# microsoft/DFOL-VQA

Hardware: AMD Instinct MI355X
Metric: questions/sec (GQA programs, N=100 objects) (higher is better)
Workload: dtype f32

## Files before the change

### dfol_vqa_amd/csrc/dfol_pair_h2.hip

```cpp
#include "dfol_common.h"
#include "dfol_split.h"

#include <stdlib.h>

#include <type_traits>

#ifdef DFOL_PAIR_TRACE
__device__ long long dfol_h2_trace_buf[8 * 8 * 64];
#define TRACE(slot)                                                                                                  \
    do {                                                                                                             \
        if (trace_on && lane == 0) dfol_h2_trace_buf[(trace_blk * 8 + wave) * 64 + (slot)] = clock64();              \
    } while (0)
#else
#define TRACE(slot)
#endif

#ifndef DFOL_H2_PREFETCH
#define DFOL_H2_PREFETCH 1
#endif
#ifndef DFOL_H2_BDEPTH
#define DFOL_H2_BDEPTH 2
#endif
#ifndef DFOL_H1_BDEPTH
#define DFOL_H1_BDEPTH 4
// ... 35 lines not shown
    return r;
}

__global__ void h2_row_scale_kernel(const float* __restrict__ W2, int64_t ld_w2, int HID2, int HID1, float* __restrict__ tail) {
    const int lane = threadIdx.x & 63, r = blockIdx.x * (blockDim.x >> 6) + (threadIdx.x >> 6);
    if (r >= H2_ROWS) return;
    float m = 0.f;
    if (r < HID2)
        for (int k = lane; k < HID1; k += 64) m = fmaxf(m, fabsf(W2[(int64_t)r * ld_w2 + k] * H2_LN2));
#pragma unroll
    for (int s = 32; s >= 1; s >>= 1) m = fmaxf(m, __shfl_xor(m, s, 64));
    const int e = dfol_scale_exp(m);
    if (lane == 0) {
        tail[r] = ldexpf(H2_NL2E, -e);
        reinterpret_cast<int32_t*>(tail)[H2_ROWS + r] = e;
    }
}

template <int NP>
__global__ void h2_pack_w2_kernel(const float* __restrict__ W2, int64_t ld_w2, int HID2, int HID1, const float* __restrict__ tail,
                                  u32x4* __restrict__ out) {
    constexpr int PIECES = NP * H2_ROWS * 4;
    const int idx = blockIdx.x * blockDim.x + threadIdx.x;
    if (idx >= (HID1 / H2_CH) * PIECES) return;
    const int c = idx / PIECES, rem = idx - c * PIECES;
    const int p = rem / (H2_ROWS * 4), rr = rem - p * H2_ROWS * 4, r = rr >> 2, slot = rr & 3;
    const int kq = slot ^ dfol_swz(r);
    const int e = reinterpret_cast<const int32_t*>(tail)[H2_ROWS + r];
    uint32_t piece[4];
#pragma unroll
    for (int j = 0; j < 4; ++j) {
        float w0 = 0.f, w1 = 0.f;
        if (r < HID2) {
            w0 = ldexpf(W2[(int64_t)r * ld_w2 + c * H2_CH + h2_kperm(kq, 2 * j)] * H2_LN2, e);
            w1 = ldexpf(W2[(int64_t)r * ld_w2 + c * H2_CH + h2_kperm(kq, 2 * j + 1)] * H2_LN2, e);
        }
        uint32_t h, l;
        dfol_split2h(w0, w1, h, l);
        piece[j] = p == 0 ? h : l;
    }
    out[idx] = u32x4{piece[0], piece[1], piece[2], piece[3]};
}

struct H2Train {
    float* Z;
    float* pre2;
    int64_t ld_pre2;
    float* geo;
    float* x;
    int64_t ld_x;
    const int64_t* pair_off;
};

template <int NB16, bool TBF16, bool TRAIN = false, int NP = 2>
__global__ __launch_bounds__(512) __attribute__((amdgpu_waves_per_eu(2, 2))) void pair_ll32h_kernel(
    const float* UV_ , int64_t ld_uv_, int HID1, const float* __restrict__ pos_, int64_t ld_pos_,
    const float* __restrict__ Wg_, const u32x4* __restrict__ W2h_, const float* __restrict__ b2_, int HID2,
    const float* __restrict__ E_, int64_t ld_e, const float* __restrict__ be, const int32_t* __restrict__ n_obj,
    const int32_t* __restrict__ obj_off, int Q, int tiles_per_image, int wg_tiles, const int32_t* __restrict__ req_col,
    const int32_t* __restrict__ req_tile, const uint8_t* __restrict__ req_orient, int K, int NS, float dflt,
    void* __restrict__ tiles_v, H2Train tr) {
    constexpr int MT = 2, WAVES = 8;
    constexpr int ROWS = NB16 * 16, T = WAVES * 64, SLOTS = MT * 16 * WAVES;
    static_assert(NB16 > 16 && NB16 <= H2_TILES, "geometry");
    static_assert(NP == 2 || (NP == 1 && !TRAIN), "pieces per operand (the train forward keeps both)");
    constexpr int PIECES = NP * H2_ROWS * 4;
    __shared__ __attribute__((aligned(16))) u32x4 Bs[2 * PIECES];
    __shared__ __attribute__((aligned(16))) u32x4 WgA[(256 / H2_CH) * 2 * 64];
    constexpr int STAGE_FLOATS = 8192;
    __shared__ __attribute__((aligned(16))) float stage[STAGE_FLOATS];

    const int wave = __builtin_amdgcn_readfirstlane((int)threadIdx.x >> 6);
#ifdef DFOL_PAIR_TRACE
    const int trace_b0 = 3000 / wg_tiles, trace_step = 500 / wg_tiles > 0 ? 500 / wg_tiles : 1;
    const int trace_blk = ((int)blockIdx.x - trace_b0) / trace_step;
    const bool trace_on = (int)blockIdx.x >= trace_b0 && ((int)blockIdx.x - trace_b0) % trace_step == 0 && trace_blk < 8;
#endif
    const int nchunk = HID1 / H2_CH, lastc = nchunk - 1;
    const int tile_end = (int)min((int64_t)blockIdx.x * wg_tiles + wg_tiles, (int64_t)Q * tiles_per_image);
    auto dma_chunk0_all = [&](const u32x4* W2h) __attribute__((always_inline)) {
        int tid = threadIdx.x;
        asm volatile("" : "+v"(tid));
#pragma unroll
        for (int i = 0; i < (PIECES + T - 1) / T; ++i)
            if (PIECES % T == 0 || T * i + wave * 64 < PIECES)
                __builtin_amdgcn_global_load_lds(W2h + T * i + tid, (__attribute__((address_space(3))) void*)&Bs[T * i + wave * 64], 16, 0, 0);
    };
    bool started = false;
    bool b0 = false;
    int stage_q = -1;
    for (int tile = (int)blockIdx.x * wg_tiles; tile < tile_end; tile = TRAIN ? tile_end : tile + 1) {
        const int q = tile / tiles_per_image, tb = tile - q * tiles_per_image;
        const int n = n_obj[q], npairs = n * (n - 1);
        if (tb * SLOTS >= npairs) continue;
        bool any = TRAIN;
        for (int k = 0; k < K; ++k) any |= req_col[(int64_t)k * Q + q] >= 0;
        if (!any) continue;
        const int64_t prow0 = TRAIN ? tr.pair_off[q] : 0;
        const u32x4* W2h = W2h_;
        const float *Wg = Wg_, *b2 = b2_, *E = E_, *UV = UV_, *pos = pos_;
        int64_t ld_uv = ld_uv_, ld_pos = ld_pos_;
        asm volatile("" : "+s"(W2h), "+s"(Wg), "+s"(b2), "+s"(E));
        asm volatile("" : "+s"(UV), "+s"(pos), "+s"(ld_uv), "+s"(ld_pos));
        int tid = threadIdx.x;
        asm volatile("" : "+v"(tid));
        const int lane = tid & 63, kh = lane >> 4, r16 = lane & 15;
        const float* cf = reinterpret_cast<const float*>(W2h + (int64_t)nchunk * PIECES);

        TRACE(0);
        if (!started) dma_chunk0_all(W2h);
        const int first = obj_off[q];
        u32x4 geoB[MT];
        const char* img_uv = reinterpret_cast<const char*>(UV + (int64_t)first * ld_uv);
        uint32_t uoff[MT], voff[MT];
        uint32_t zoff[MT];
        auto slot_geometry = [&]() __attribute__((always_inline)) {
#pragma unroll
            for (int m = 0; m < MT; ++m) {
                const int e_slot = tb * SLOTS + wave * (MT * 16) + m * 16 + r16;
                const bool valid = e_slot < npairs;
                zoff[m] = (TRAIN && valid) ? (uint32_t)(e_slot * HID1 + 4 * kh) * 4u : 0xffffffffu;
                const int s = valid ? e_slot / (n - 1) : 0, oo_ = valid ? e_slot - s * (n - 1) : 0, o = oo_ + (oo_ >= s);
                const float4 g = dfol_pair_geometry(pos + (int64_t)(first + s) * ld_pos, pos + (int64_t)(first + o) * ld_pos);
                uint32_t gh01, gl01, gh23, gl23;
                dfol_split2h(g.x, g.y, gh01, gl01);
                dfol_split2h(g.z, g.w, gh23, gl23);
                if (TRAIN && valid && kh == 0) *reinterpret_cast<floatx4*>(tr.geo + (prow0 + e_slot) * 4) = floatx4{g.x, g.y, g.z, g.w};
                geoB[m] = kh == 0 ? u32x4{gh01, gh23, gl01, gl23} : (kh == 1 ? u32x4{gh01, gh23, 0u, 0u} : u32x4{0u, 0u, 0u, 0u});
                uoff[m] = (uint32_t)(s * (int)ld_uv + 4 * kh) * 4u;
                voff[m] = (uint32_t)(o * (int)ld_uv + HID1 + 4 * kh) * 4u;
            }
        };
        constexpr int SR = STAGE_FLOATS / ROWS - 2;
        const int Kc = K < SR ? K : SR;
        floatx4 acc[MT][NB16];
#pragma unroll
        for (int m = 0; m < MT; ++m)
#pragma unroll
            for (int i = 0; i < NB16; ++i) acc[m][i] = floatx4{0.f, 0.f, 0.f, 0.f};

        auto dma_chunk = [&](int c, int buf, int w, int ln) __attribute__((always_inline)) {
            constexpr int PER_WAVE = PIECES / 4;
            const u32x4* src = W2h + (int64_t)c * PIECES + w * PER_WAVE + ln;
            u32x4* dst = &Bs[buf * PIECES + w * PER_WAVE];
#pragma unroll
            for (int g = 0; g < PER_WAVE / 64; g += 4) {
#if DFOL_H2_DMA_ASM
                const uint32_t d = (uint32_t)(uintptr_t)(__attribute__((address_space(3))) void*)(dst + 64 * g);
                const u32x4* sp = src + 64 * g;
#pragma clang diagnostic push
#pragma clang diagnostic ignored "-Winline-asm"
                const uint32_t m0v = __builtin_amdgcn_readfirstlane(d);
                const int rem = PER_WAVE / 64 - g;
                if (rem >= 4)
                    asm volatile("s_mov_b32 m0, %1\n\ts_nop 0\n\tglobal_load_lds_dwordx4 %0, off\n\tglobal_load_lds_dwordx4 %0, off offset:1024\n\t"
                                 "global_load_lds_dwordx4 %0, off offset:2048\n\tglobal_load_lds_dwordx4 %0, off offset:3072" ::"v"(sp), "s"(m0v) : "memory", "m0");
                else if (rem == 3)
                    asm volatile("s_mov_b32 m0, %1\n\ts_nop 0\n\tglobal_load_lds_dwordx4 %0, off\n\tglobal_load_lds_dwordx4 %0, off offset:1024\n\t"
                                 "global_load_lds_dwordx4 %0, off offset:2048" ::"v"(sp), "s"(m0v) : "memory", "m0");
                else if (rem == 2)
                    asm volatile("s_mov_b32 m0, %1\n\ts_nop 0\n\tglobal_load_lds_dwordx4 %0, off\n\tglobal_load_lds_dwordx4 %0, off offset:1024" ::"v"(sp), "s"(m0v) : "memory", "m0");
                else
                    asm volatile("s_mov_b32 m0, %1\n\ts_nop 0\n\tglobal_load_lds_dwordx4 %0, off" ::"v"(sp), "s"(m0v) : "memory", "m0");
#pragma clang diagnostic pop
#else
                auto d = (__attribute__((address_space(3))) void*)(dst + 64 * g);
                __builtin_amdgcn_global_load_lds(src + 64 * g, d, 16, 0, 0);
                if (g + 1 < PER_WAVE / 64) __builtin_amdgcn_global_load_lds(src + 64 * g, d, 16, 1024, 0);
                if (g + 2 < PER_WAVE / 64) __builtin_amdgcn_global_load_lds(src + 64 * g, d, 16, 2048, 0);
                if (g + 3 < PER_WAVE / 64) __builtin_amdgcn_global_load_lds(src + 64 * g, d, 16, 3072, 0);
#endif
            }
        };
        floatx4 ru[MT][2], rv[MT][2];
        auto load_uv = [&](int c) __attribute__((always_inline)) {
            const char* base = img_uv + (uint32_t)__builtin_amdgcn_readfirstlane(H2_CH * 4 * c);
#pragma unroll
            for (int m = 0; m < MT; ++m)
#pragma unroll
                for (int half = 0; half < 2; ++half) {
                    ru[m][half] = *reinterpret_cast<const floatx4*>(base + uoff[m] + 64 * half);
                    rv[m][half] = *reinterpret_cast<const floatx4*>(base + voff[m] + 64 * half);
                }
        };
        u32x4 ap[MT][NP];
        auto make_a = [&](int c) __attribute__((always_inline)) {
            floatx4 z[MT][2];
#pragma unroll
            for (int t = 0; t < 2; ++t) {
                const f16x8 wa = __builtin_bit_cast(f16x8, WgA[(2 * c + t) * 64 + lane]);
#pragma unroll
                for (int m = 0; m < MT; ++m)
                    z[m][t] = __builtin_amdgcn_mfma_f32_16x16x32_f16(wa, __builtin_bit_cast(f16x8, geoB[m]), ru[m][t] + rv[m][t], 0, 0, 0);
            }
#pragma unroll
            for (int m = 0; m < MT; ++m)
#pragma unroll
                for (int t = 0; t < 2; ++t)
#pragma unroll
                    for (int jp = 0; jp < 2; ++jp) {
                        const float z0 = z[m][t][2 * jp], z1 = z[m][t][2 * jp + 1];
                        const float a0 = __builtin_amdgcn_fmed3f(z0, h2_elu_neg(z0), H2_AMAX);
                        const float a1 = __builtin_amdgcn_fmed3f(z1, h2_elu_neg(z1), H2_AMAX);
                        const uint32_t hh = __builtin_bit_cast(uint32_t, __builtin_convertvector((f32x2){a0, a1}, f16x2));
                        ap[m][0][2 * t + jp] = hh;
                        if constexpr (NP == 2)
                            ap[m][1][2 * t + jp] = __builtin_bit_cast(uint32_t, __builtin_convertvector((f32x2){h2_resid<false>(a0, hh), h2_resid<true>(a1, hh)}, f16x2));
                        if (TRAIN) z[m][t][2 * jp] = a0 * H2_LN2, z[m][t][2 * jp + 1] = a1 * H2_LN2;
                    }
            if (TRAIN && !(DFOL_H2T_SKIP & 1)) {
                char* zimg = reinterpret_cast<char*>(tr.Z + prow0 * HID1) + (uint32_t)__builtin_amdgcn_readfirstlane(H2_CH * 4 * c);
#pragma unroll
                for (int m = 0; m < MT; ++m)
                    if (zoff[m] != 0xffffffffu) {
#pragma unroll
                        for (int t = 0; t < 2; ++t) *reinterpret_cast<floatx4*>(zimg + zoff[m] + 64 * t) = z[m][t];
                    }
            }
        };
        const int boff = r16 * 4 + (kh ^ dfol_swz(r16));
        int bbase = boff;
        auto load_b = [&](int i, f16x8 (&b)[NP]) __attribute__((always_inline)) {
#pragma unroll
            for (int p = 0; p < NP; ++p) b[p] = __builtin_bit_cast(f16x8, Bs[bbase + i * 64 + p * H2_ROWS * 4]);
        };
        constexpr int PA3[3] = {1, 0, 0}, PB3[3] = {0, 1, 0};
        auto chunk_mfma = [&]() __attribute__((always_inline)) {
            constexpr int D = NP == 2 ? DFOL_H2_BDEPTH : DFOL_H1_BDEPTH;
            f16x8 bq[D + 1][NP];
#pragma unroll
            for (int d = 0; d < D; ++d) load_b(d, bq[d]);
#pragma unroll
            for (int i = 0; i < NB16; ++i) {
                if (i + D < NB16) load_b(i + D, bq[(i + D) % (D + 1)]);
                __builtin_amdgcn_sched_barrier(0);
#pragma unroll
                for (int m = 0; m < MT; ++m) {
#pragma unroll
                    for (int x = NP == 2 ? 0 : 2; x < 3; ++x)
                        acc[m][i] = __builtin_amdgcn_mfma_f32_16x16x32_f16(__builtin_bit_cast(f16x8, ap[m][PA3[x]]), bq[i % (D + 1)][PB3[x]], acc[m][i], 0, 0, 0);
                    __builtin_amdgcn_sched_barrier(0);
                }
            }
        };
        slot_geometry();
        if (started) {
            __syncthreads();
            if (!b0) dma_chunk0_all(W2h);
        } else {
            int tid = threadIdx.x;
            asm volatile("" : "+v"(tid));
            for (int i = tid; i < (HID1 / 16) * 64; i += T) {
                const int kt = i >> 6, ln = i & 63, khh = ln >> 4;
                u32x4 frag = {0u, 0u, 0u, 0u};
                if (khh < 2) {
                    const float4 g = *reinterpret_cast<const float4*>(Wg + (kt * 16 + (ln & 15)) * 4);
                    uint32_t h01, l01, h23, l23;
                    dfol_split2h(g.x * H2_L2E, g.y * H2_L2E, h01, l01);
                    dfol_split2h(g.z * H2_L2E, g.w * H2_L2E, h23, l23);
                    frag = khh == 0 ? u32x4{h01, h23, h01, h23} : u32x4{l01, l23, 0u, 0u};
                }
                WgA[i] = frag;
            }
        }
        if (q != stage_q) {
            int tid = threadIdx.x;
            asm volatile("" : "+v"(tid));
            for (int i = tid; i < ROWS; i += T) {
                stage[i] = H2_NL2E * (i < HID2 ? b2[i] : -1.0e30f);
                stage[ROWS + i] = i < HID2 ? cf[i] : 0.f;
            }
            for (int k = 0; k < Kc; ++k) {
                const int col = req_col[(int64_t)k * Q + q];
                for (int i = tid; i < ROWS; i += T) stage[ROWS * (2 + k) + i] = (col >= 0 && i < HID2) ? E[(int64_t)col * ld_e + i] : 0.f;
            }
        }
        __builtin_amdgcn_s_waitcnt(0x0F70);
        __syncthreads();

        const bool pf = (lastc & 1) && tile + 1 < tile_end;
        auto run_half = [&](auto y_tag) __attribute__((always_inline)) {
            constexpr bool Y = decltype(y_tag)::value;
            TRACE(1);
            if (Y) {
                if (nchunk > 1) dma_chunk(1, 1, wave - 4, lane);
                if (DFOL_H2_PREFETCH) load_uv(0);
                __syncthreads();
            } else if (DFOL_H2_PREFETCH) {
                load_uv(0);
            }
            TRACE(2);
            for (int c = 0; c < nchunk; ++c) {
                if (!DFOL_H2_PREFETCH) load_uv(c);
                if (DFOL_H2_PREFETCH) {
                    floatx4 t0 = ru[0][0], t1 = ru[0][1], t2 = ru[1][0], t3 = ru[1][1], t4 = rv[0][0], t5 = rv[0][1], t6 = rv[1][0], t7 = rv[1][1];
                    asm volatile("s_waitcnt vmcnt(0)" : "+v"(t0), "+v"(t1), "+v"(t2), "+v"(t3), "+v"(t4), "+v"(t5), "+v"(t6), "+v"(t7));
                    ru[0][0] = t0, ru[0][1] = t1, ru[1][0] = t2, ru[1][1] = t3, rv[0][0] = t4, rv[0][1] = t5, rv[1][0] = t6, rv[1][1] = t7;
                }
                TRACE(40 + c);
                if (Y && !DFOL_H2_DMA_LATE && c >= 1 && c < lastc) dma_chunk(c + 1, (c + 1) & 1, wave - 4, lane);
                TRACE(50 + c);
                make_a(c);
#pragma unroll
                for (int m = 0; m < MT; ++m)
#pragma unroll
                    for (int p = 0; p < NP; ++p) asm volatile("" : "+v"(ap[m][p]));
                __builtin_amdgcn_sched_barrier(0);
                if (Y && DFOL_H2_DMA_LATE && c >= 1 && c < lastc) dma_chunk(c + 1, (c + 1) & 1, wave - 4, lane);
                TRACE(3 + 4 * c);
                __syncthreads();
                __builtin_amdgcn_sched_barrier(0);
                TRACE(4 + 4 * c);
                bbase = boff + (c & 1) * PIECES;
                if (DFOL_H2_PREFETCH && c < lastc) load_uv(c + 1);
                chunk_mfma();
                if (Y) __builtin_amdgcn_s_waitcnt(0x0F70);
                TRACE(5 + 4 * c);
                if (!Y || c < lastc) __syncthreads();
                TRACE(6 + 4 * c);
            }
            if (!Y && pf) {
                int ln = lane;
                asm volatile("" : "+v"(ln));
                dma_chunk(0, 0, wave, ln);
            }
        };
        if (wave < 4) run_half(std::false_type());
        else run_half(std::true_type());

        const int64_t tile_sz = (int64_t)NS * NS;
#pragma unroll
        for (int m = 0; m < MT; ++m)
#pragma unroll
            for (int i = 0; i < NB16; ++i) {
                const float bv = stage[i * 16 + r16], cm = stage[ROWS + i * 16 + r16];
                if (TRAIN && !(DFOL_H2T_SKIP & 2)) {
                    const int colp = i * 16 + r16;
#pragma unroll
                    for (int e = 0; e < 4; ++e) {
                        const int ee = tb * SLOTS + wave * (MT * 16) + m * 16 + 4 * kh + e;
                        if (colp < HID2 && ee < npairs)
                            *reinterpret_cast<float*>(reinterpret_cast<char*>(tr.pre2 + prow0 * tr.ld_pre2) + (uint32_t)(ee * (int)tr.ld_pre2 + colp) * 4u) =
                                -H2_LN2 * fmaf(acc[m][i][e], cm, bv);
                    }
                }
#pragma unroll
                for (int e = 0; e < 4; ++e) acc[m][i][e] = __builtin_amdgcn_rcpf(1.0f + __builtin_amdgcn_exp2f(fmaf(acc[m][i][e], cm, bv)));
            }
        for (int k = 0; k < K; ++k) {
            const int col = req_col[(int64_t)k * Q + q];
            if (col < 0) continue;
            float vm[MT];
#pragma unroll
            for (int m = 0; m < MT; ++m) {
                float part[4] = {0.f, 0.f, 0.f, 0.f};
                if (k < Kc) {
                    const float* erow = stage + ROWS * (2 + k) + r16;
#pragma unroll
                    for (int i = 0; i < NB16; ++i) {
                        const float ev = erow[i * 16];
#pragma unroll
                        for (int e = 0; e < 4; ++e) part[e] = fmaf(acc[m][i][e], ev, part[e]);
                    }
                } else {
                    const float* erow = E + (int64_t)col * ld_e;
                    int c16 = r16;
                    asm volatile("" : "+v"(c16));
#pragma unroll
                    for (int i = 0; i < NB16; ++i) {
                        const float ev = erow[min(i * 16 + c16, HID2 - 1)];
#pragma unroll
                        for (int e = 0; e < 4; ++e) part[e] = fmaf(acc[m][i][e], ev, part[e]);
                    }
                }
#pragma unroll
                for (int e = 0; e < 4; ++e) part[e] = dfol_group_sum<16>(part[e]);
                vm[m] = r16 == 0 ? part[0] : (r16 == 1 ? part[1] : (r16 == 2 ? part[2] : part[3]));
            }
            const float shifted = __int_as_float(__builtin_amdgcn_update_dpp(0, __float_as_int(vm[1]), 0x114, 0xF, 0xF, false));
            if (r16 < 8) {
                const int hi = r16 >> 2;
                const float v = hi ? shifted : vm[0];
                const int ee = tb * SLOTS + wave * (MT * 16) + hi * 16 + 4 * kh + (r16 & 3);
                if (ee < npairs) {
                    if (TRAIN) {
                        tr.x[(int64_t)k * tr.ld_x + prow0 + ee] = v;
                        continue;
                    }
                    int ss, oo;
                    dfol_offdiag_slot_rcp(ee, n, ss, oo);
                    const float x = v + (be ? be[col] : 0.f);
                    const float val = fminf(x, 0.f) - dfol_log(1.0f + dfol_exp(-fabsf(x)));
                    const int64_t at = (int64_t)req_tile[(int64_t)k * Q + q] * tile_sz +
                                       ((req_orient && req_orient[(int64_t)k * Q + q]) ? (int64_t)oo * NS + ss : (int64_t)ss * NS + oo);
                    if (TBF16) {
                        uint32_t u = __float_as_uint(val);
                        u += 0x7fffu + ((u >> 16) & 1u);
                        reinterpret_cast<uint16_t*>(tiles_v)[at] = (uint16_t)(u >> 16);
                    } else {
                        reinterpret_cast<float*>(tiles_v)[at] = val;
                    }
                }
            }
        }
        TRACE(60);
        started = true;
        stage_q = q;
        b0 = pf;
    }
    __builtin_amdgcn_s_waitcnt(0x0F70);
}

__global__ __launch_bounds__(512) void h2_uv_range_kernel(const float* __restrict__ UV, int64_t ld_uv, int HID1, const float* __restrict__ pos,
                                                          int64_t ld_pos, const float* __restrict__ Wg, const int32_t* __restrict__ n_obj,
                                                          const int32_t* __restrict__ obj_off, uint32_t* __restrict__ status) {
    __shared__ float4 part[512];
    __shared__ float box[4][8];
    const int q = blockIdx.x, n = n_obj[q], first = obj_off[q], t = threadIdx.x, lane = t & 63, wave = t >> 6;
    if (n < 2) return;
    const int G = (2 * HID1) / 4, R = 512 / G, cg = t % G, rg = t / G;
    float4 m = {-INFINITY, -INFINITY, -INFINITY, -INFINITY};
    bool nan = false;
    const float* base = UV + (int64_t)first * ld_uv + 4 * cg;
    auto take = [&](const float4 a) {
        nan |= (a.x != a.x) | (a.y != a.y) | (a.z != a.z) | (a.w != a.w);
        m.x = fmaxf(m.x, a.x), m.y = fmaxf(m.y, a.y), m.z = fmaxf(m.z, a.z), m.w = fmaxf(m.w, a.w);
    };
    int o = rg;
    for (; o + 3 * R < n; o += 4 * R) {
        const float4 a = *reinterpret_cast<const float4*>(base + (int64_t)o * ld_uv), b = *reinterpret_cast<const float4*>(base + (int64_t)(o + R) * ld_uv);
        const float4 c = *reinterpret_cast<const float4*>(base + (int64_t)(o + 2 * R) * ld_uv), d = *reinterpret_cast<const float4*>(base + (int64_t)(o + 3 * R) * ld_uv);
        take(a), take(b), take(c), take(d);
    }
    for (; o < n; o += R) take(*reinterpret_cast<const float4*>(base + (int64_t)o * ld_uv));
    if (nan) m.x = NAN;
    part[t] = m;
    float lox = INFINITY, hix = -INFINITY, loy = INFINITY, hiy = -INFINITY;
    for (int i = t; i < n; i += 512) {
        const float* p = pos + (int64_t)(first + i) * ld_pos;
        const float cx = p[0] + p[2] / 2.0f, cy = p[1] + p[3] / 2.0f;
        lox = fminf(lox, cx), hix = fmaxf(hix, cx), loy = fminf(loy, cy), hiy = fmaxf(hiy, cy);
    }
#pragma unroll
    for (int s = 32; s >= 1; s >>= 1) {
        lox = fminf(lox, __shfl_xor(lox, s, 64)), hix = fmaxf(hix, __shfl_xor(hix, s, 64));
        loy = fminf(loy, __shfl_xor(loy, s, 64)), hiy = fmaxf(hiy, __shfl_xor(hiy, s, 64));
    }
    if (lane == 0) box[0][wave] = lox, box[1][wave] = hix, box[2][wave] = loy, box[3][wave] = hiy;
    __syncthreads();
    if (t < HID1) {
#pragma unroll
        for (int w = 0; w < 8; ++w) lox = fminf(lox, box[0][w]), hix = fmaxf(hix, box[1][w]), loy = fminf(loy, box[2][w]), hiy = fmaxf(hiy, box[3][w]);
        const float* pf = reinterpret_cast<const float*>(part);
        float mu = -INFINITY, mv = -INFINITY;
        bool bad = false;
        for (int r = 0; r < R; ++r) {
            const float u = pf[(r * G + t / 4) * 4 + (t & 3)], v = pf[(r * G + (HID1 + t) / 4) * 4 + (t & 3)];
            const float ux = pf[(r * G + t / 4) * 4], vx = pf[(r * G + (HID1 + t) / 4) * 4];
            bad |= (ux != ux) | (vx != vx);
            mu = fmaxf(mu, u), mv = fmaxf(mv, v);
        }
        const float dmax = sqrtf((hix - lox) * (hix - lox) + (hiy - loy) * (hiy - loy));
        const float4 g = *reinterpret_cast<const float4*>(Wg + t * 4);
        const float geo = H2_L2E * (fabsf(g.x) * dmax + fabsf(g.y) * 1.57079632679489661923f + fabsf(g.z) + fabsf(g.w));
        const float bound = mu + mv + geo;
// ... 156 lines not shown
        }
        __syncthreads();
        for (int j = 0; j < n_ent; ++j) {
            const int first = __builtin_amdgcn_readfirstlane(ent[2][j]), end = __builtin_amdgcn_readfirstlane(ent[3][j]);
            if (end <= w0 || first >= w0 + MT * 16) continue;
            const int p = __builtin_amdgcn_readfirstlane(ent[0][j]), col = __builtin_amdgcn_readfirstlane(ent[1][j]);
            float vm[MT];
#pragma unroll
            for (int m = 0; m < MT; ++m) {
                float part[4] = {0.f, 0.f, 0.f, 0.f};
                if (j < SR) {
                    const float* erow = stage + ROWS * (2 + j) + r16;
#pragma unroll
                    for (int i = 0; i < NB16; ++i) {
                        const float ev = erow[i * 16];
#pragma unroll
                        for (int e = 0; e < 4; ++e) part[e] = fmaf(acc[m][i][e], ev, part[e]);
                    }
                } else {
                    const float* erow = E + (int64_t)col * ld_e;
#pragma unroll
                    for (int i = 0; i < NB16; ++i) {
                        const float ev = i * 16 + r16 < HID2 ? erow[i * 16 + r16] : 0.f;
#pragma unroll
                        for (int e = 0; e < 4; ++e) part[e] = fmaf(acc[m][i][e], ev, part[e]);
                    }
                }
#pragma unroll
                for (int e = 0; e < 4; ++e) part[e] = dfol_group_sum<16>(part[e]);
                vm[m] = r16 == 0 ? part[0] : (r16 == 1 ? part[1] : (r16 == 2 ? part[2] : part[3]));
            }
            const float shifted = __int_as_float(__builtin_amdgcn_update_dpp(0, __float_as_int(vm[1]), 0x114, 0xF, 0xF, false));
            if (r16 < 8) {
                const int hi = r16 >> 2;
                const int g = w0 + hi * 16 + 4 * kh + (r16 & 3);
                if (g >= first && g < end && g - first < NS) {
                    const float x = (hi ? shifted : vm[0]) + (be ? be[col] : 0.f);
                    ll[(int64_t)p * NS + (g - first)] = fminf(x, 0.f) - log1pf(expf(-fabsf(x)));
                }
            }
        }
    }
}

}

#ifdef DFOL_PAIR_TRACE
extern "C" int dfol_pair_h2_trace_read(long long* out) { return (int)hipMemcpyFromSymbol(out, HIP_SYMBOL(dfol_h2_trace_buf), sizeof(dfol_h2_trace_buf)); }
#endif

#ifndef DFOL_H2_WG_TILES
#define DFOL_H2_WG_TILES 4
#endif
static int h2_wg_tiles() {
    const char* e = getenv("DFOL_PAIR_TILES");
    const int t = e ? atoi(e) : DFOL_H2_WG_TILES;
    return t < 1 ? 1 : (t > 64 ? 64 : t);
}

extern "C" int64_t dfol_pair_w2_f16x2_bytes(int32_t HID1) { return (int64_t)(HID1 / H2_CH) * H2_PIECES * 16 + 2 * H2_ROWS * 4; }
extern "C" int64_t dfol_pair_w2_f16_bytes(int32_t HID1) { return (int64_t)(HID1 / H2_CH) * H1_PIECES * 16 + 2 * H2_ROWS * 4; }

template <int NP>
static int h2_pack_w2(const char* name, const float* W2, int64_t ld_w2, int32_t HID2, int32_t HID1, void* W2_split, void* stream) {
    DFOL_REQUIRE(HID1 > 0 && HID1 <= 256 && HID1 % H2_CH == 0, "%s: HID1=%d must be a multiple of %d, <= 256", name, HID1, H2_CH);
    DFOL_REQUIRE(HID2 > 256 && HID2 <= 320, "%s: HID2=%d must be in (256, 320]", name, HID2);
    DFOL_REQUIRE(W2 && W2_split && ld_w2 >= HID1, "%s: null pointer or ld_w2 < HID1", name);
    DFOL_REQUIRE((uintptr_t)W2_split % 16 == 0, "%s: output must be 16-byte aligned", name);
    const int total = (HID1 / H2_CH) * NP * H2_ROWS * 4;
    float* tail = reinterpret_cast<float*>(reinterpret_cast<u32x4*>(W2_split) + total);
    hipLaunchKernelGGL(h2_row_scale_kernel, dim3(H2_ROWS / 4), dim3(256), 0, (hipStream_t)stream, W2, ld_w2, HID2, HID1, tail);
    hipLaunchKernelGGL(h2_pack_w2_kernel<NP>, dim3(dfol_cdiv(total, 256)), dim3(256), 0, (hipStream_t)stream, W2, ld_w2, HID2, HID1, (const float*)tail,
                       (u32x4*)W2_split);
    DFOL_LAUNCH_CHECK(name);
    return 0;
}

extern "C" int dfol_pair_pack_w2_f16x2(const float* W2, int64_t ld_w2, int32_t HID2, int32_t HID1, void* W2_split, void* stream) {
    return h2_pack_w2<2>("pair_pack_w2_f16x2", W2, ld_w2, HID2, HID1, W2_split, stream);
}

extern "C" int dfol_pair_pack_w2_f16(const float* W2, int64_t ld_w2, int32_t HID2, int32_t HID1, void* W2_split, void* stream) {
    return h2_pack_w2<1>("pair_pack_w2_f16", W2, ld_w2, HID2, HID1, W2_split, stream);
}

template <int NP>
static int h2_pair_ll(const char* name, const float* UV, int64_t ld_uv, int32_t HID1, const float* pos, int64_t ld_pos, const float* Wg,
                      const void* W2_split, const float* b2, int32_t HID2, const float* E, int64_t ld_e, const float* be, const int32_t* n_obj,
                      const int32_t* obj_off, int32_t Q, int32_t max_n, const int32_t* req_col, const int32_t* req_tile, const uint8_t* req_orient,
                      int32_t K, int32_t NS, float default_ll, int32_t tile_dtype, void* tiles_v, void* stream) {
    DFOL_REQUIRE(tile_dtype == DFOL_TILE_F32 || (tile_dtype == DFOL_TILE_BF16 && NS % 8 == 0), "%s: tile_dtype=%d (bf16 tiles need NS %% 8 == 0)", name, tile_dtype);
    DFOL_REQUIRE(Q >= 0 && K >= 0 && NS > 0 && NS % 4 == 0 && max_n >= 0 && max_n <= NS, "%s: bad sizes Q=%d K=%d NS=%d max_n=%d", name, Q, K, NS, max_n);
    DFOL_REQUIRE(HID1 > 0 && HID1 <= 256 && HID1 % H2_CH == 0 && ld_uv % 4 == 0, "%s: HID1=%d must be a multiple of %d, <= 256, UV rows 16-byte aligned", name, HID1, H2_CH);
    DFOL_REQUIRE(HID2 > 256 && HID2 <= 320, "%s: HID2=%d must be in (256, 320]", name, HID2);
    DFOL_REQUIRE(max_n <= DFOL_OFFDIAG_RCP_MAX_N, "%s: max_n=%d is above %d objects per image, the range of the epilogue's reciprocal pair decode (dfol_common.h)",
                 name, max_n, DFOL_OFFDIAG_RCP_MAX_N);
    if (Q == 0 || K == 0 || max_n < 2) return 0;
    DFOL_REQUIRE(UV && pos && Wg && W2_split && b2 && E && n_obj && obj_off && req_col && req_tile && tiles_v, "%s: null pointer", name);
    DFOL_REQUIRE(((uintptr_t)UV % 16 == 0) && ((uintptr_t)W2_split % 16 == 0) && ((uintptr_t)Wg % 16 == 0), "%s: operands must be 16-byte aligned", name);
    hipStream_t st = (hipStream_t)stream;
    const int tpi = dfol_cdiv((int64_t)max_n * (max_n - 1), 256);
    DFOL_REQUIRE((int64_t)Q * tpi < ((int64_t)1 << 31), "%s: too many tiles", name);
    DFOL_REQUIRE((int64_t)max_n * ld_uv * 4 < ((int64_t)1 << 31), "%s: an image's U / V rows must span less than 2 GB", name);
    const int wgt = h2_wg_tiles();
    const dim3 grid((unsigned)dfol_cdiv((int64_t)Q * tpi, wgt));
    if (uint32_t* status = dfol_range_status_ptr())
        hipLaunchKernelGGL(h2_uv_range_kernel, dim3((unsigned)Q), dim3(512), 0, st, UV, ld_uv, HID1, pos, ld_pos, Wg, n_obj, obj_off, status);
    const H2Train none = {nullptr, nullptr, 0, nullptr, nullptr, 0, nullptr};
#define DFOL_PAIR32H(NBV, BF)                                                                                                       \
    hipLaunchKernelGGL((pair_ll32h_kernel<NBV, BF, false, NP>), grid, dim3(512), 0, st, UV, ld_uv, HID1, pos, ld_pos, Wg, (const u32x4*)W2_split, b2, HID2, \
                       E, ld_e, be, n_obj, obj_off, Q, tpi, wgt, req_col, req_tile, req_orient, K, NS, default_ll, tiles_v, none)
    if (HID2 <= 272) { if (tile_dtype == DFOL_TILE_BF16) DFOL_PAIR32H(17, true); else DFOL_PAIR32H(17, false); }
    else if (HID2 <= 288) { if (tile_dtype == DFOL_TILE_BF16) DFOL_PAIR32H(18, true); else DFOL_PAIR32H(18, false); }
    else if (HID2 <= 304) { if (tile_dtype == DFOL_TILE_BF16) DFOL_PAIR32H(19, true); else DFOL_PAIR32H(19, false); }
    else { if (tile_dtype == DFOL_TILE_BF16) DFOL_PAIR32H(20, true); else DFOL_PAIR32H(20, false); }
#undef DFOL_PAIR32H
    DFOL_LAUNCH_CHECK(name);
    return 0;
}

extern "C" int dfol_pair_ll_h2_f32(const float* UV, int64_t ld_uv, int32_t HID1, const float* pos, int64_t ld_pos, const float* Wg,
                                   const void* W2_split, const float* b2, int32_t HID2, const float* E, int64_t ld_e,
                                   const float* be, const int32_t* n_obj, const int32_t* obj_off, int32_t Q, int32_t max_n,
                                   const int32_t* req_col, const int32_t* req_tile, const uint8_t* req_orient, int32_t K,
                                   int32_t NS, float default_ll, int32_t tile_dtype, void* tiles_v, void* stream) {
    return h2_pair_ll<2>("pair_ll_h2", UV, ld_uv, HID1, pos, ld_pos, Wg, W2_split, b2, HID2, E, ld_e, be, n_obj, obj_off, Q, max_n, req_col, req_tile, req_orient, K,
                         NS, default_ll, tile_dtype, tiles_v, stream);
}

extern "C" int dfol_pair_ll_h1_f32(const float* UV, int64_t ld_uv, int32_t HID1, const float* pos, int64_t ld_pos, const float* Wg,
                                   const void* W2_f16, const float* b2, int32_t HID2, const float* E, int64_t ld_e,
                                   const float* be, const int32_t* n_obj, const int32_t* obj_off, int32_t Q, int32_t max_n,
                                   const int32_t* req_col, const int32_t* req_tile, const uint8_t* req_orient, int32_t K,
                                   int32_t NS, float default_ll, int32_t tile_dtype, void* tiles_v, void* stream) {
    return h2_pair_ll<1>("pair_ll_h1", UV, ld_uv, HID1, pos, ld_pos, Wg, W2_f16, b2, HID2, E, ld_e, be, n_obj, obj_off, Q, max_n, req_col, req_tile, req_orient, K,
                         NS, default_ll, tile_dtype, tiles_v, stream);
}


extern "C" int dfol_pair_train_fwd_h2_f32(const float* UV, int64_t ld_uv, int32_t HID1, const float* pos, int64_t ld_pos, const float* Wg,
                                          const void* W2_split, const float* b2, int32_t HID2, const float* E, int64_t ld_e, const int32_t* n_obj,
                                          const int32_t* obj_off, const int64_t* pair_off, int32_t Q, int32_t max_n, const int32_t* req_row, int32_t K,
                                          float* Z, float* pre2, int64_t ld_pre2, float* geo, float* x, int64_t ld_x, void* stream) {
    DFOL_REQUIRE(Q >= 0 && K >= 0 && max_n >= 0, "pair_train_fwd_h2: bad sizes Q=%d K=%d max_n=%d", Q, K, max_n);
    DFOL_REQUIRE(HID1 > 0 && HID1 <= 256 && HID1 % H2_CH == 0 && ld_uv % 4 == 0, "pair_train_fwd_h2: HID1=%d must be a multiple of %d, <= 256, UV rows 16-byte aligned", HID1, H2_CH);
    DFOL_REQUIRE(HID2 > 256 && HID2 <= 320 && ld_pre2 >= HID2, "pair_train_fwd_h2: HID2=%d must be in (256, 320], ld_pre2 >= HID2", HID2);
    if (Q == 0 || max_n < 2) return 0;
    DFOL_REQUIRE(UV && pos && Wg && W2_split && b2 && n_obj && obj_off && pair_off && Z && pre2 && geo && (K == 0 || (E && req_row && x)), "pair_train_fwd_h2: null pointer");
    DFOL_REQUIRE(((uintptr_t)UV % 16 == 0) && ((uintptr_t)W2_split % 16 == 0) && ((uintptr_t)Wg % 16 == 0) && ((uintptr_t)Z % 16 == 0) && ((uintptr_t)geo % 16 == 0),
                 "pair_train_fwd_h2: operands must be 16-byte aligned");
    hipStream_t st = (hipStream_t)stream;
    const int tpi = dfol_cdiv((int64_t)max_n * (max_n - 1), 256);
    DFOL_REQUIRE((int64_t)Q * tpi < ((int64_t)1 << 31), "pair_train_fwd_h2: too many tiles");
    DFOL_REQUIRE((int64_t)max_n * ld_uv * 4 < ((int64_t)1 << 31) && (int64_t)max_n * (max_n - 1) * HID1 * 4 < ((int64_t)1 << 32) - 1,
                 "pair_train_fwd_h2: an image's rows must span less than 2 GB (U | V) / 4 GB (Z)");
    if (uint32_t* status = dfol_range_status_ptr())
        hipLaunchKernelGGL(h2_uv_range_kernel, dim3((unsigned)Q), dim3(512), 0, st, UV, ld_uv, HID1, pos, ld_pos, Wg, n_obj, obj_off, status);
    const H2Train tr = {Z, pre2, ld_pre2, geo, x, ld_x, pair_off};
    const int wgt = 1;
    const dim3 grid((unsigned)Q * tpi);
#define DFOL_PAIR32T(NBV)                                                                                                                    \
    hipLaunchKernelGGL((pair_ll32h_kernel<NBV, false, true>), grid, dim3(512), 0, st, UV, ld_uv, HID1, pos, ld_pos, Wg, (const u32x4*)W2_split, b2, HID2, \
                       E, ld_e, (const float*)nullptr, n_obj, obj_off, Q, tpi, wgt, req_row, (const int32_t*)nullptr, (const uint8_t*)nullptr, K, 4, 0.f,      \
                       (void*)nullptr, tr)
// ... 35 lines not shown
```

Baseline: 195,100.

## Add 4-wavefront pair kernel with three-slot half-chunk W2 ring

Adds a 4-wave (256-thread) form of the pair kernel for two-piece inference. Every wave now computes all output columns and streams W2 through a three-slot ring of half-chunks, so the next half's DMA overlaps the MFMA on the current one and counted waits replace full drains. Tiles shrink to 128 pairs, the default tiles per workgroup rises to 8, and the launcher picks this form by default through a new DFOL_PAIR_WG setting. The intent is higher occupancy with less LDS and fewer idle waves per workgroup. The cost is more barriers per chunk and a much smaller stage buffer (fewer K columns staged at once).

```diff
diff --git a/dfol_vqa_amd/csrc/dfol_pair_h2.hip b/dfol_vqa_amd/csrc/dfol_pair_h2.hip
--- a/dfol_vqa_amd/csrc/dfol_pair_h2.hip
+++ b/dfol_vqa_amd/csrc/dfol_pair_h2.hip
@@ -111,22 +111,25 @@
     const int64_t* pair_off;
 };
 
-template <int NB16, bool TBF16, bool TRAIN = false, int NP = 2>
-__global__ __launch_bounds__(512) __attribute__((amdgpu_waves_per_eu(2, 2))) void pair_ll32h_kernel(
+template <int NB16, bool TBF16, bool TRAIN = false, int NP = 2, int WAVES = 8>
+__global__ __launch_bounds__(WAVES * 64) __attribute__((amdgpu_waves_per_eu(2, 2))) void pair_ll32h_kernel(
     const float* UV_ , int64_t ld_uv_, int HID1, const float* __restrict__ pos_, int64_t ld_pos_,
     const float* __restrict__ Wg_, const u32x4* __restrict__ W2h_, const float* __restrict__ b2_, int HID2,
     const float* __restrict__ E_, int64_t ld_e, const float* __restrict__ be, const int32_t* __restrict__ n_obj,
     const int32_t* __restrict__ obj_off, int Q, int tiles_per_image, int wg_tiles, const int32_t* __restrict__ req_col,
     const int32_t* __restrict__ req_tile, const uint8_t* __restrict__ req_orient, int K, int NS, float dflt,
     void* __restrict__ tiles_v, H2Train tr) {
-    constexpr int MT = 2, WAVES = 8;
+    constexpr int MT = 2;
+    constexpr bool QUAD = WAVES == 4;
     constexpr int ROWS = NB16 * 16, T = WAVES * 64, SLOTS = MT * 16 * WAVES;
     static_assert(NB16 > 16 && NB16 <= H2_TILES, "geometry");
     static_assert(NP == 2 || (NP == 1 && !TRAIN), "pieces per operand (the train forward keeps both)");
+    static_assert(WAVES == 8 || (QUAD && NP == 2 && !TRAIN), "the 4-wavefront form: two-piece inference");
     constexpr int PIECES = NP * H2_ROWS * 4;
-    __shared__ __attribute__((aligned(16))) u32x4 Bs[2 * PIECES];
+    constexpr int HROWS = H2_ROWS / 2, HTILES = H2_TILES / 2, HPIECES = PIECES / 2;
+    __shared__ __attribute__((aligned(16))) u32x4 Bs[QUAD ? 3 * HPIECES : 2 * PIECES];
     __shared__ __attribute__((aligned(16))) u32x4 WgA[(256 / H2_CH) * 2 * 64];
-    constexpr int STAGE_FLOATS = 8192;
+    constexpr int STAGE_FLOATS = QUAD ? 1024 : 8192;
     __shared__ __attribute__((aligned(16))) float stage[STAGE_FLOATS];
 
     const int wave = __builtin_amdgcn_readfirstlane((int)threadIdx.x >> 6);
@@ -147,6 +150,7 @@
     };
     bool started = false;
     bool b0 = false;
+    int ring = 0;
     int stage_q = -1;
     for (int tile = (int)blockIdx.x * wg_tiles; tile < tile_end; tile = TRAIN ? tile_end : tile + 1) {
         const int q = tile / tiles_per_image, tb = tile - q * tiles_per_image;
@@ -166,51 +170,17 @@
         const int lane = tid & 63, kh = lane >> 4, r16 = lane & 15;
         const float* cf = reinterpret_cast<const float*>(W2h + (int64_t)nchunk * PIECES);
 
-        TRACE(0);
-        if (!started) dma_chunk0_all(W2h);
-        const int first = obj_off[q];
-        u32x4 geoB[MT];
-        const char* img_uv = reinterpret_cast<const char*>(UV + (int64_t)first * ld_uv);
-        uint32_t uoff[MT], voff[MT];
-        uint32_t zoff[MT];
-        auto slot_geometry = [&]() __attribute__((always_inline)) {
-#pragma unroll
-            for (int m = 0; m < MT; ++m) {
-                const int e_slot = tb * SLOTS + wave * (MT * 16) + m * 16 + r16;
-                const bool valid = e_slot < npairs;
-                zoff[m] = (TRAIN && valid) ? (uint32_t)(e_slot * HID1 + 4 * kh) * 4u : 0xffffffffu;
-                const int s = valid ? e_slot / (n - 1) : 0, oo_ = valid ? e_slot - s * (n - 1) : 0, o = oo_ + (oo_ >= s);
-                const float4 g = dfol_pair_geometry(pos + (int64_t)(first + s) * ld_pos, pos + (int64_t)(first + o) * ld_pos);
-                uint32_t gh01, gl01, gh23, gl23;
-                dfol_split2h(g.x, g.y, gh01, gl01);
-                dfol_split2h(g.z, g.w, gh23, gl23);
-                if (TRAIN && valid && kh == 0) *reinterpret_cast<floatx4*>(tr.geo + (prow0 + e_slot) * 4) = floatx4{g.x, g.y, g.z, g.w};
-                geoB[m] = kh == 0 ? u32x4{gh01, gh23, gl01, gl23} : (kh == 1 ? u32x4{gh01, gh23, 0u, 0u} : u32x4{0u, 0u, 0u, 0u});
-                uoff[m] = (uint32_t)(s * (int)ld_uv + 4 * kh) * 4u;
-                voff[m] = (uint32_t)(o * (int)ld_uv + HID1 + 4 * kh) * 4u;
-            }
-        };
-        constexpr int SR = STAGE_FLOATS / ROWS - 2;
-        const int Kc = K < SR ? K : SR;
-        floatx4 acc[MT][NB16];
-#pragma unroll
-        for (int m = 0; m < MT; ++m)
-#pragma unroll
-            for (int i = 0; i < NB16; ++i) acc[m][i] = floatx4{0.f, 0.f, 0.f, 0.f};
-
-        auto dma_chunk = [&](int c, int buf, int w, int ln) __attribute__((always_inline)) {
-            constexpr int PER_WAVE = PIECES / 4;
-            const u32x4* src = W2h + (int64_t)c * PIECES + w * PER_WAVE + ln;
-            u32x4* dst = &Bs[buf * PIECES + w * PER_WAVE];
-#pragma unroll
-            for (int g = 0; g < PER_WAVE / 64; g += 4) {
+        auto dma_run = [&](const u32x4* src, u32x4* dst, auto nreq_tag) __attribute__((always_inline)) {
+            constexpr int NREQ = decltype(nreq_tag)::value;
+#pragma unroll
+            for (int g = 0; g < NREQ; g += 4) {
 #if DFOL_H2_DMA_ASM
                 const uint32_t d = (uint32_t)(uintptr_t)(__attribute__((address_space(3))) void*)(dst + 64 * g);
                 const u32x4* sp = src + 64 * g;
 #pragma clang diagnostic push
 #pragma clang diagnostic ignored "-Winline-asm"
                 const uint32_t m0v = __builtin_amdgcn_readfirstlane(d);
-                const int rem = PER_WAVE / 64 - g;
+                const int rem = NREQ - g;
                 if (rem >= 4)
                     asm volatile("s_mov_b32 m0, %1\n\ts_nop 0\n\tglobal_load_lds_dwordx4 %0, off\n\tglobal_load_lds_dwordx4 %0, off offset:1024\n\t"
                                  "global_load_lds_dwordx4 %0, off offset:2048\n\tglobal_load_lds_dwordx4 %0, off offset:3072" ::"v"(sp), "s"(m0v) : "memory", "m0");
@@ -225,12 +195,62 @@
 #else
                 auto d = (__attribute__((address_space(3))) void*)(dst + 64 * g);
                 __builtin_amdgcn_global_load_lds(src + 64 * g, d, 16, 0, 0);
-                if (g + 1 < PER_WAVE / 64) __builtin_amdgcn_global_load_lds(src + 64 * g, d, 16, 1024, 0);
-                if (g + 2 < PER_WAVE / 64) __builtin_amdgcn_global_load_lds(src + 64 * g, d, 16, 2048, 0);
-                if (g + 3 < PER_WAVE / 64) __builtin_amdgcn_global_load_lds(src + 64 * g, d, 16, 3072, 0);
-#endif
-            }
-        };
+                if (g + 1 < NREQ) __builtin_amdgcn_global_load_lds(src + 64 * g, d, 16, 1024, 0);
+                if (g + 2 < NREQ) __builtin_amdgcn_global_load_lds(src + 64 * g, d, 16, 2048, 0);
+                if (g + 3 < NREQ) __builtin_amdgcn_global_load_lds(src + 64 * g, d, 16, 3072, 0);
+#endif
+            }
+        };
+        auto dma_chunk = [&](int c, int buf, int w, int ln) __attribute__((always_inline)) {
+            constexpr int PER_WAVE = PIECES / 4;
+            dma_run(W2h + (int64_t)c * PIECES + w * PER_WAVE + ln, &Bs[buf * PIECES + w * PER_WAVE], std::integral_constant<int, PER_WAVE / 64>());
+        };
+        constexpr int DMA_HALF_REQS = HPIECES / 4 / 64;
+        auto dma_half = [&](int c, int h, int slot, int ln) __attribute__((always_inline)) {
+            if constexpr (QUAD) {
+                static_assert(HPIECES % (4 * 64) == 0 && DMA_HALF_REQS == 5, "a wavefront's share of a half-chunk: whole requests");
+                const int sub = (wave & 1) * (HPIECES / 4);
+                dma_run(W2h + (int64_t)c * PIECES + (wave >> 1) * (H2_ROWS * 4) + h * (HROWS * 4) + sub + ln,
+                        &Bs[slot * HPIECES + (wave >> 1) * (HROWS * 4) + sub], std::integral_constant<int, DMA_HALF_REQS>());
+            }
+        };
+        auto request_first = [&]() __attribute__((always_inline)) {
+            if constexpr (QUAD) dma_half(0, 0, ring, lane);
+            else dma_chunk0_all(W2h);
+        };
+
+        TRACE(0);
+        if (!started) request_first();
+        const int first = obj_off[q];
+        u32x4 geoB[MT];
+        const char* img_uv = reinterpret_cast<const char*>(UV + (int64_t)first * ld_uv);
+        uint32_t uoff[MT], voff[MT];
+        uint32_t zoff[MT];
+        auto slot_geometry = [&]() __attribute__((always_inline)) {
+#pragma unroll
+            for (int m = 0; m < MT; ++m) {
+                const int e_slot = tb * SLOTS + wave * (MT * 16) + m * 16 + r16;
+                const bool valid = e_slot < npairs;
+                zoff[m] = (TRAIN && valid) ? (uint32_t)(e_slot * HID1 + 4 * kh) * 4u : 0xffffffffu;
+                const int s = valid ? e_slot / (n - 1) : 0, oo_ = valid ? e_slot - s * (n - 1) : 0, o = oo_ + (oo_ >= s);
+                const float4 g = dfol_pair_geometry(pos + (int64_t)(first + s) * ld_pos, pos + (int64_t)(first + o) * ld_pos);
+                uint32_t gh01, gl01, gh23, gl23;
+                dfol_split2h(g.x, g.y, gh01, gl01);
+                dfol_split2h(g.z, g.w, gh23, gl23);
+                if (TRAIN && valid && kh == 0) *reinterpret_cast<floatx4*>(tr.geo + (prow0 + e_slot) * 4) = floatx4{g.x, g.y, g.z, g.w};
+                geoB[m] = kh == 0 ? u32x4{gh01, gh23, gl01, gl23} : (kh == 1 ? u32x4{gh01, gh23, 0u, 0u} : u32x4{0u, 0u, 0u, 0u});
+                uoff[m] = (uint32_t)(s * (int)ld_uv + 4 * kh) * 4u;
+                voff[m] = (uint32_t)(o * (int)ld_uv + HID1 + 4 * kh) * 4u;
+            }
+        };
+        constexpr int SR = STAGE_FLOATS / ROWS - 2;
+        const int Kc = K < SR ? K : SR;
+        floatx4 acc[MT][NB16];
+#pragma unroll
+        for (int m = 0; m < MT; ++m)
+#pragma unroll
+            for (int i = 0; i < NB16; ++i) acc[m][i] = floatx4{0.f, 0.f, 0.f, 0.f};
+
         floatx4 ru[MT][2], rv[MT][2];
         auto load_uv = [&](int c) __attribute__((always_inline)) {
             const char* base = img_uv + (uint32_t)__builtin_amdgcn_readfirstlane(H2_CH * 4 * c);
@@ -279,19 +299,25 @@
         };
         const int boff = r16 * 4 + (kh ^ dfol_swz(r16));
         int bbase = boff;
+        int bbase1 = boff;
         auto load_b = [&](int i, f16x8 (&b)[NP]) __attribute__((always_inline)) {
 #pragma unroll
-            for (int p = 0; p < NP; ++p) b[p] = __builtin_bit_cast(f16x8, Bs[bbase + i * 64 + p * H2_ROWS * 4]);
+            for (int p = 0; p < NP; ++p) {
+                if constexpr (QUAD) b[p] = __builtin_bit_cast(f16x8, Bs[(i < HTILES ? bbase : bbase1) + (i % HTILES) * 64 + p * HROWS * 4]);
+                else b[p] = __builtin_bit_cast(f16x8, Bs[bbase + i * 64 + p * H2_ROWS * 4]);
+            }
         };
         constexpr int PA3[3] = {1, 0, 0}, PB3[3] = {0, 1, 0};
-        auto chunk_mfma = [&]() __attribute__((always_inline)) {
+        auto chunk_mfma = [&](auto i0_tag, auto i1_tag) __attribute__((always_inline)) {
+            constexpr int I0 = decltype(i0_tag)::value, I1 = decltype(i1_tag)::value;
             constexpr int D = NP == 2 ? DFOL_H2_BDEPTH : DFOL_H1_BDEPTH;
+            static_assert(I1 - I0 >= D, "fragment prefetch depth");
             f16x8 bq[D + 1][NP];
 #pragma unroll
-            for (int d = 0; d < D; ++d) load_b(d, bq[d]);
-#pragma unroll
-            for (int i = 0; i < NB16; ++i) {
-                if (i + D < NB16) load_b(i + D, bq[(i + D) % (D + 1)]);
+            for (int d = 0; d < D; ++d) load_b(I0 + d, bq[(I0 + d) % (D + 1)]);
+#pragma unroll
+            for (int i = I0; i < I1; ++i) {
+                if (i + D < I1) load_b(i + D, bq[(i + D) % (D + 1)]);
                 __builtin_amdgcn_sched_barrier(0);
 #pragma unroll
                 for (int m = 0; m < MT; ++m) {
@@ -305,7 +331,7 @@
         slot_geometry();
         if (started) {
             __syncthreads();
-            if (!b0) dma_chunk0_all(W2h);
+            if (!b0) request_first();
         } else {
             int tid = threadIdx.x;
             asm volatile("" : "+v"(tid));
@@ -337,7 +363,20 @@
         __builtin_amdgcn_s_waitcnt(0x0F70);
         __syncthreads();
 
-        const bool pf = (lastc & 1) && tile + 1 < tile_end;
+        const bool pf = (QUAD || (lastc & 1)) && tile + 1 < tile_end;
+        auto wait_uv = [&]() __attribute__((always_inline)) {
+            floatx4 t0 = ru[0][0], t1 = ru[0][1], t2 = ru[1][0], t3 = ru[1][1], t4 = rv[0][0], t5 = rv[0][1], t6 = rv[1][0], t7 = rv[1][1];
+            asm volatile("s_waitcnt vmcnt(0)" : "+v"(t0), "+v"(t1), "+v"(t2), "+v"(t3), "+v"(t4), "+v"(t5), "+v"(t6), "+v"(t7));
+            ru[0][0] = t0, ru[0][1] = t1, ru[1][0] = t2, ru[1][1] = t3, rv[0][0] = t4, rv[0][1] = t5, rv[1][0] = t6, rv[1][1] = t7;
+        };
+        auto build_a = [&](int c) __attribute__((always_inline)) {
+            make_a(c);
+#pragma unroll
+            for (int m = 0; m < MT; ++m)
+#pragma unroll
+                for (int p = 0; p < NP; ++p) asm volatile("" : "+v"(ap[m][p]));
+            __builtin_amdgcn_sched_barrier(0);
+        };
         auto run_half = [&](auto y_tag) __attribute__((always_inline)) {
             constexpr bool Y = decltype(y_tag)::value;
             TRACE(1);
@@ -351,20 +390,11 @@
             TRACE(2);
             for (int c = 0; c < nchunk; ++c) {
                 if (!DFOL_H2_PREFETCH) load_uv(c);
-                if (DFOL_H2_PREFETCH) {
-                    floatx4 t0 = ru[0][0], t1 = ru[0][1], t2 = ru[1][0], t3 = ru[1][1], t4 = rv[0][0], t5 = rv[0][1], t6 = rv[1][0], t7 = rv[1][1];
-                    asm volatile("s_waitcnt vmcnt(0)" : "+v"(t0), "+v"(t1), "+v"(t2), "+v"(t3), "+v"(t4), "+v"(t5), "+v"(t6), "+v"(t7));
-                    ru[0][0] = t0, ru[0][1] = t1, ru[1][0] = t2, ru[1][1] = t3, rv[0][0] = t4, rv[0][1] = t5, rv[1][0] = t6, rv[1][1] = t7;
-                }
+                if (DFOL_H2_PREFETCH) wait_uv();
                 TRACE(40 + c);
                 if (Y && !DFOL_H2_DMA_LATE && c >= 1 && c < lastc) dma_chunk(c + 1, (c + 1) & 1, wave - 4, lane);
                 TRACE(50 + c);
-                make_a(c);
-#pragma unroll
-                for (int m = 0; m < MT; ++m)
-#pragma unroll
-                    for (int p = 0; p < NP; ++p) asm volatile("" : "+v"(ap[m][p]));
-                __builtin_amdgcn_sched_barrier(0);
+                build_a(c);
                 if (Y && DFOL_H2_DMA_LATE && c >= 1 && c < lastc) dma_chunk(c + 1, (c + 1) & 1, wave - 4, lane);
                 TRACE(3 + 4 * c);
                 __syncthreads();
@@ -372,7 +402,7 @@
                 TRACE(4 + 4 * c);
                 bbase = boff + (c & 1) * PIECES;
                 if (DFOL_H2_PREFETCH && c < lastc) load_uv(c + 1);
-                chunk_mfma();
+                chunk_mfma(std::integral_constant<int, 0>(), std::integral_constant<int, NB16>());
                 if (Y) __builtin_amdgcn_s_waitcnt(0x0F70);
                 TRACE(5 + 4 * c);
                 if (!Y || c < lastc) __syncthreads();
@@ -384,7 +414,47 @@
                 dma_chunk(0, 0, wave, ln);
             }
         };
-        if (wave < 4) run_half(std::false_type());
+        auto run_quad = [&](auto) __attribute__((always_inline)) {
+            TRACE(1);
+            load_uv(0);
+            TRACE(2);
+            for (int c = 0; c < nchunk; ++c) {
+                const int s1 = ring == 2 ? 0 : ring + 1, s2 = ring == 0 ? 2 : ring - 1;
+                wait_uv();
+                TRACE(40 + c);
+                {
+                    int ln = lane;
+                    asm volatile("" : "+v"(ln));
+                    dma_half(c, 1, s1, ln);
+                }
+                TRACE(50 + c);
+                build_a(c);
+                TRACE(3 + 4 * c);
+                __builtin_amdgcn_s_barrier();
+                __builtin_amdgcn_sched_barrier(0);
+                TRACE(4 + 4 * c);
+                bbase = boff + ring * HPIECES, bbase1 = boff + s1 * HPIECES;
+                if (c < lastc || pf) {
+                    int ln = lane;
+                    asm volatile("" : "+v"(ln));
+                    dma_half(c < lastc ? c + 1 : 0, 0, s2, ln);
+                }
+                __builtin_amdgcn_sched_barrier(0);
+                chunk_mfma(std::integral_constant<int, 0>(), std::integral_constant<int, HTILES>());
+                static_assert(DMA_HALF_REQS == 5, "the counted wait below");
+                if (c < lastc || pf) __builtin_amdgcn_s_waitcnt(0x0F75);
+                else __builtin_amdgcn_s_waitcnt(0x0F70);
+                TRACE(5 + 4 * c);
+                __builtin_amdgcn_s_barrier();
+                __builtin_amdgcn_sched_barrier(0);
+                TRACE(6 + 4 * c);
+                if (c < lastc) load_uv(c + 1);
+                chunk_mfma(std::integral_constant<int, HTILES>(), std::integral_constant<int, NB16>());
+                ring = s2;
+            }
+        };
+        if constexpr (QUAD) run_quad(0);
+        else if (wave < 4) run_half(std::false_type());
         else run_half(std::true_type());
 
         const int64_t tile_sz = (int64_t)NS * NS;
@@ -470,6 +540,9 @@
     __builtin_amdgcn_s_waitcnt(0x0F70);
 }
 
+template <int NB16, bool TBF16, int NP = 2>
+constexpr auto pair_ll32q_kernel = pair_ll32h_kernel<NB16, TBF16, false, NP, 4>;
+
 __global__ __launch_bounds__(512) void h2_uv_range_kernel(const float* __restrict__ UV, int64_t ld_uv, int HID1, const float* __restrict__ pos,
                                                           int64_t ld_pos, const float* __restrict__ Wg, const int32_t* __restrict__ n_obj,
                                                           const int32_t* __restrict__ obj_off, uint32_t* __restrict__ status) {
@@ -732,10 +805,21 @@
 #ifndef DFOL_H2_WG_TILES
 #define DFOL_H2_WG_TILES 4
 #endif
-static int h2_wg_tiles() {
+#ifndef DFOL_H2Q_WG_TILES
+#define DFOL_H2Q_WG_TILES 8
+#endif
+static int h2_wg_tiles(bool quad) {
     const char* e = getenv("DFOL_PAIR_TILES");
-    const int t = e ? atoi(e) : DFOL_H2_WG_TILES;
+    const int t = e ? atoi(e) : (quad ? DFOL_H2Q_WG_TILES : DFOL_H2_WG_TILES);
     return t < 1 ? 1 : (t > 64 ? 64 : t);
+}
+#ifndef DFOL_H2_PAIR_WG
+#define DFOL_H2_PAIR_WG 4
+#endif
+static int h2_pair_wg() {
+    const char* e = getenv("DFOL_PAIR_WG");
+    const int w = e ? atoi(e) : DFOL_H2_PAIR_WG;
+    return w == 8 ? 8 : (w == 4 ? 4 : DFOL_H2_PAIR_WG);
 }
 
 extern "C" int64_t dfol_pair_w2_f16x2_bytes(int32_t HID1) { return (int64_t)(HID1 / H2_CH) * H2_PIECES * 16 + 2 * H2_ROWS * 4; }
@@ -779,17 +863,27 @@
     DFOL_REQUIRE(UV && pos && Wg && W2_split && b2 && E && n_obj && obj_off && req_col && req_tile && tiles_v, "%s: null pointer", name);
     DFOL_REQUIRE(((uintptr_t)UV % 16 == 0) && ((uintptr_t)W2_split % 16 == 0) && ((uintptr_t)Wg % 16 == 0), "%s: operands must be 16-byte aligned", name);
     hipStream_t st = (hipStream_t)stream;
-    const int tpi = dfol_cdiv((int64_t)max_n * (max_n - 1), 256);
+    const bool quad = NP == 2 && h2_pair_wg() == 4;
+    const int tpi = dfol_cdiv((int64_t)max_n * (max_n - 1), quad ? 128 : 256);
     DFOL_REQUIRE((int64_t)Q * tpi < ((int64_t)1 << 31), "%s: too many tiles", name);
     DFOL_REQUIRE((int64_t)max_n * ld_uv * 4 < ((int64_t)1 << 31), "%s: an image's U / V rows must span less than 2 GB", name);
-    const int wgt = h2_wg_tiles();
+    const int wgt = h2_wg_tiles(quad);
     const dim3 grid((unsigned)dfol_cdiv((int64_t)Q * tpi, wgt));
     if (uint32_t* status = dfol_range_status_ptr())
         hipLaunchKernelGGL(h2_uv_range_kernel, dim3((unsigned)Q), dim3(512), 0, st, UV, ld_uv, HID1, pos, ld_pos, Wg, n_obj, obj_off, status);
     const H2Train none = {nullptr, nullptr, 0, nullptr, nullptr, 0, nullptr};
 #define DFOL_PAIR32H(NBV, BF)                                                                                                       \
-    hipLaunchKernelGGL((pair_ll32h_kernel<NBV, BF, false, NP>), grid, dim3(512), 0, st, UV, ld_uv, HID1, pos, ld_pos, Wg, (const u32x4*)W2_split, b2, HID2, \
-                       E, ld_e, be, n_obj, obj_off, Q, tpi, wgt, req_col, req_tile, req_orient, K, NS, default_ll, tiles_v, none)
+    do {                                                                                                                            \
+        if constexpr (NP == 2) {                                                                                                    \
+            if (quad) {                                                                                                             \
+                hipLaunchKernelGGL((pair_ll32q_kernel<NBV, BF, 2>), grid, dim3(256), 0, st, UV, ld_uv, HID1, pos, ld_pos, Wg, (const u32x4*)W2_split, b2, HID2, \
+                                   E, ld_e, be, n_obj, obj_off, Q, tpi, wgt, req_col, req_tile, req_orient, K, NS, default_ll, tiles_v, none);                  \
+                break;                                                                                                              \
+            }                                                                                                                       \
+        }                                                                                                                           \
+        hipLaunchKernelGGL((pair_ll32h_kernel<NBV, BF, false, NP>), grid, dim3(512), 0, st, UV, ld_uv, HID1, pos, ld_pos, Wg, (const u32x4*)W2_split, b2, HID2, \
+                           E, ld_e, be, n_obj, obj_off, Q, tpi, wgt, req_col, req_tile, req_orient, K, NS, default_ll, tiles_v, none);                          \
+    } while (0)
     if (HID2 <= 272) { if (tile_dtype == DFOL_TILE_BF16) DFOL_PAIR32H(17, true); else DFOL_PAIR32H(17, false); }
     else if (HID2 <= 288) { if (tile_dtype == DFOL_TILE_BF16) DFOL_PAIR32H(18, true); else DFOL_PAIR32H(18, false); }
     else if (HID2 <= 304) { if (tile_dtype == DFOL_TILE_BF16) DFOL_PAIR32H(19, true); else DFOL_PAIR32H(19, false); }
```

Result: slower. 189,200 (-3.0%).
